# XUANTIE-RV/csi-nn2

Hardware: AMD Instinct MI355X
Metric: mobilenetv1_int8_images_per_sec (higher is better)
Workload: dtype i8; 1 GPU; mobilenetv1 int8 NHWC batch 1/GPU, 28 conv layers in 15 launches, hipGraph replay via csinn_*; ops_per_image=1137480704, algorithmic_bytes_per_image=8323144, algorithmic_bytes_per_image_survey=14444616, parallelism=replicas x1

## Files before the change

csi-nn2_amd/__init__.py:

```python
import ctypes as C
import os

import numpy as np

HERE = os.path.dirname(os.path.abspath(__file__))
ROOT = os.path.dirname(HERE)
LIB_DIR = os.path.join(HERE, "lib")

DTYPE_INT8, DTYPE_INT32, DTYPE_FLOAT16, DTYPE_FLOAT32 = 3, 7, 8, 10
MEM_CPU, MEM_DMABUF, MEM_CPU_ACC = 0, 2, 5
QUANT_INT8_ASYM_W_SYM, QUANT_FLOAT16 = 11, 7
API_REF, API_GREF, API_MI355X = 0, 1, 14
RM_LAYER, RM_CPU_GRAPH = 0, 1
LAYOUT_N, LAYOUT_NC, LAYOUT_NCHW, LAYOUT_O, LAYOUT_OI, LAYOUT_OIHW, LAYOUT_O1HW = 1, 2, 4, 6, 7, 11, 13
LAYOUT_NHWC, LAYOUT_OHWI, LAYOUT_1HWO = 15, 18, 22
CSINN_TRUE = 1
OP_CONV2D, OP_CONV2D_RELU, OP_CONV2D_RELU6 = 28, 29, 30
OP_DEPTHWISE_CONV2D, OP_FULLYCONNECTED = 35, 71

SHL_NHWC, SHL_NCHW = 0, 1
SHL_I8, SHL_F16 = 0, 1
ACT_NONE, ACT_RELU, ACT_RELU6 = 0, 1, 2
ALGO_AUTO, ALGO_DIRECT, ALGO_IGEMM, ALGO_DW, ALGO_GEMV, ALGO_STEM = 0, 1, 2, 3, 4, 5

# ... 155 lines not shown
        "shl_mi355x_comm_unique_id": (C.c_int, [vp]),
        "shl_mi355x_comm_create": (C.c_int, [vp, i32, i32, C.POINTER(vp)]),
        "shl_mi355x_comm_destroy": (C.c_int, [vp]),
        "shl_mi355x_comm_info": (C.c_int, [vp, C.POINTER(i32), C.POINTER(i32), C.POINTER(i32)]),
        "shl_mi355x_device_bus_id": (C.c_int, [C.c_char_p, sz]),
        "shl_mi355x_comm_bcast": (C.c_int, [vp, C.POINTER(vp), C.POINTER(sz), i32, i32, vp]),
        "shl_mi355x_conv_plan_destroy": (C.c_int, [vp]),
        "shl_mi355x_conv_plan_algo": (C.c_int, [vp]),
        "shl_mi355x_conv_plan_kernel_name": (C.c_char_p, [vp]),
        "shl_mi355x_conv_plan_bytes": (sz, [vp]),
        "shl_mi355x_conv_plan_const_block": (vp, [vp, C.POINTER(sz)]),
        "shl_mi355x_conv_plan_adopt_block": (C.c_int, [vp, vp]),
        "shl_mi355x_conv_forward": (C.c_int, [vp, vp, vp, i32, vp]),
        "shl_mi355x_pwdw_fusable": (C.c_int, [vp, vp, i32]),
        "shl_mi355x_pwdw_form": (C.c_int, [vp, vp, i32]),
        "shl_mi355x_pool_conv_fusable": (C.c_int, [vp, i32, i32]),
        "shl_mi355x_pool_conv_forward": (C.c_int, [vp, vp, vp, i32, i32, f32, i32, f32, i32, vp]),
        "shl_mi355x_conv_pool_fusable": (C.c_int, [vp, i32]),
        "shl_mi355x_conv_pool_forward": (C.c_int, [vp, vp, vp, vp, i32, f32, i32, f32, i32, vp]),
        "shl_mi355x_conv_plan_set_no_stream_consumer": (C.c_int, [vp, i32]),
        "shl_mi355x_pwdw_forward": (C.c_int, [vp, vp, vp, vp, i32, vp]),
        "shl_mi355x_relu_i8": (C.c_int, [vp, vp, sz, f32, i32, f32, i32, i32, vp]),
        "shl_mi355x_relu_f16": (C.c_int, [vp, vp, sz, i32, vp]),
        "shl_mi355x_add": (C.c_int, [vp, vp, vp, sz, i32, f32, i32, f32, i32, f32, i32, vp]),
        "shl_mi355x_layout_convert": (C.c_int, [vp, vp, C.c_int64, i32, i32, i32, i32, vp]),
        "shl_mi355x_global_avgpool2d": (C.c_int, [vp, vp, i32, i32, i32, i32, i32, f32, i32, f32, i32, vp]),
        "shl_mi355x_softmax": (C.c_int, [vp, vp, i32, C.c_int64, i32, C.c_int64, f32, i32, f32, i32, vp]),
    }
    for name, (res, args) in sigs.items():
        fn = getattr(lib, name)
# ... 213 lines not shown
```

csi-nn2_amd/csrc/common.h:

```cpp
#pragma once

#include <hip/hip_runtime.h>
#include <stdint.h>

#include "shl_mi355x.h"

namespace shl {

typedef int v4i __attribute__((ext_vector_type(4)));
typedef int v16i __attribute__((ext_vector_type(16)));
typedef float v16f __attribute__((ext_vector_type(16)));
typedef _Float16 v8h __attribute__((ext_vector_type(8)));

struct ConvArgs {
    const void *in;
    const void *w;
    void *out;
    const int32_t *acc_init;
    const float *mult;
    const float *bias;
    int32_t N, H, W, C;
    int32_t Ho, Wo, Co;
    int32_t Kh, Kw;
    int32_t sh, sw, pt, pl, dh, dw;
// ... 423 lines not shown
int launch_dwconv_channel(const ConvArgs &a, hipStream_t s);
bool conv_gemv_pick(const ConvArgs &a, int esize);
int launch_conv_gemv(const ConvArgs &a, int dtype, hipStream_t s);
bool pool_gemv_pick(const ConvArgs &a, int hw);
int launch_pool_gemv(const ConvArgs &a, int hw, float in_scale, int in_zp, float mid_scale, int mid_zp, hipStream_t s);
bool stem_supports(const shl_mi355x_conv_desc &d);
void stem_pack_weights(const shl_mi355x_conv_desc &d, const int8_t *ohwi, int32_t *dst);
size_t stem_weight_bytes(const shl_mi355x_conv_desc &d);
int launch_conv_stem(const ConvArgs &a, hipStream_t s);
bool conv1x1_nchw_eligible(const ConvArgs &a);
int launch_conv1x1_nchw(const ConvArgs &a, int dtype, hipStream_t s);
bool dwconv_nchw_supports(const shl_mi355x_conv_desc &d);
int launch_dwconv_nchw(const ConvArgs &a, int dtype, hipStream_t s);
bool pwdw_fusable(const ConvArgs &pw, const ConvArgs &dw, int pw_is_igemm, int dw_dot4_packed);
int launch_pwdw_fused(const ConvArgs &pw, const ConvArgs &dw, hipStream_t s);
bool stemdw_f16_nchw_fusable(const ConvArgs &stem, const ConvArgs &dw);
int launch_stemdw_f16_nchw(const ConvArgs &stem, const ConvArgs &dw, hipStream_t s);
bool stem_mfma_pick(const ConvArgs &a);
bool dwpw_stream_fusable(const ConvArgs &dw, const ConvArgs &pw, int dw_dot4_packed, int pw_is_igemm);
bool dwpw_stream_takes(const ConvArgs &dw);
int launch_dwpw_stream(const ConvArgs &dw, const ConvArgs &pw, hipStream_t s);
bool dwpw_resident_fusable(const ConvArgs &dw, const ConvArgs &pw, int dw_dot4_packed, int pw_is_igemm);
bool dwpw_resident_takes(const ConvArgs &dw);
int launch_dwpw_resident(const ConvArgs &dw, const ConvArgs &pw, hipStream_t s);
bool pwdw_f16_nchw_fusable(const ConvArgs &pw, const ConvArgs &dw);
int launch_pwdw_f16_nchw(const ConvArgs &pw, const ConvArgs &dw, hipStream_t s);
bool stemdw_fusable(const ConvArgs &stem, const ConvArgs &dw);
int launch_stemdw_fused(const ConvArgs &stem, const ConvArgs &dw, hipStream_t s);
bool patch_supports(const shl_mi355x_conv_desc &d);
int patch_choose_geom(const shl_mi355x_conv_desc &d, int32_t batch);
// ... 9 lines not shown
```

csi-nn2_amd/csrc/conv_plan.hip:

```cpp
#include <stdlib.h>
#include <string.h>

#include <map>
#include <mutex>
#include <vector>

#include "igemm_common.h"

struct shl_mi355x_conv_plan {
    shl_mi355x_conv_desc desc;
    int algo;
    char *block;
    size_t block_bytes;
    size_t off_w, off_acc, off_mult, off_bias, off_pad;
    size_t off_wfrag;
    size_t off_wpatch;
    size_t off_flags;
    int32_t pt_geom;
    int32_t div_exact, div_fma, act_clamp;
    float clamp_lo, clamp_hi, inv_out_scale;
    char *scratch_in, *scratch_out;
    int2 *pix_tab;
    float ch_in_scale, ch_out_scale;
    int32_t ch_has_bias;
// ... 984 lines not shown
    const bool i8_nhwc = pw->desc.dtype == SHL_MI355X_I8 && pw->desc.layout == SHL_MI355X_NHWC;
    const bool f16_nchw = pw->desc.dtype == SHL_MI355X_F16 && pw->desc.layout == SHL_MI355X_NCHW;
    if (!i8_nhwc && !f16_nchw) return 0;
    ConvArgs a, b;
    static char dummy[16];
    if (fill_args(pw, dummy, dummy, batch, a) != SHL_MI355X_OK || fill_args(dw, dummy, dummy, batch, b) != SHL_MI355X_OK)
        return 0;
    return pwdw_kernel_for(pw, dw, a, b);
}

int shl_mi355x_pwdw_fusable(const shl_mi355x_conv_plan *pw, const shl_mi355x_conv_plan *dw, int32_t batch)
{
    return shl_mi355x_pwdw_form(pw, dw, batch) ? 1 : 0;
}

int shl_mi355x_pwdw_forward(const shl_mi355x_conv_plan *pw, const shl_mi355x_conv_plan *dw, const void *input_dev,
                            void *output_dev, int32_t batch, void *stream)
{
    if (!dw || !pw || !input_dev || !output_dev) {
        set_error("pwdw_forward: NULL argument");
        return SHL_MI355X_EINVAL;
    }
    if (!shl_mi355x_pwdw_fusable(pw, dw, batch)) {
        set_error("pwdw_forward: the pair does not qualify for the fused kernel");
        return SHL_MI355X_ENOTSUP;
    }
    ConvArgs a, b;
    int rc = fill_args(pw, input_dev, output_dev, batch, a);
    if (rc == SHL_MI355X_OK) rc = fill_args(dw, input_dev, output_dev, batch, b);
    if (rc != SHL_MI355X_OK) return rc;
// ... 13 lines not shown
```

csi-nn2_amd/csrc/dw_patch.h:

```cpp
#pragma once

#include <stddef.h>

#include "common.h"

namespace shl {

__device__ __forceinline__ int dw_patch_slot(int j, int group, int pitch) { return group * pitch + j; }
__host__ __device__ __forceinline__ int dw_patch_pitch(int npx) { return ((npx + 31) & ~31) + 8; }
__host__ __device__ __forceinline__ size_t dw_patch_bytes(int npx) { return (size_t)dw_patch_pitch(npx) * 32; }
__device__ __forceinline__ uint32_t dw_patch_pad(const ConvArgs &d) { return (uint32_t)(d.in_zp & 0xff) * 0x01010101u; }

template <class T>
__device__ __forceinline__ T kernarg_here(size_t off)
{
    typedef const __attribute__((address_space(4))) char *KernargPtr;
    KernargPtr p = (KernargPtr)__builtin_amdgcn_kernarg_segment_ptr();
    asm volatile("" : "+s"(p));
    T v;
    __builtin_memcpy(&v, (const __attribute__((address_space(4))) T *)(p + off), sizeof(T));
    return v;
}

struct DwPatchGeom {
    int bh, bw;
    int rw;
    int pitch;
    uint32_t bw_magic;
    int oy0, ox0;
    int ry0, rx0;
    int n;
    int ch0;
};

struct DwThreadConsts {
    uint4 w0, w1, w2;
    int4 ai;
    float4 mu, bi;
};

// ... 18 lines not shown
struct DwPrep {
    int8_t *out_img;
    int nout;
    int po;
    DwOutPos first;
};

__device__ __forceinline__ DwOutPos dw_patch_locate(const ConvArgs &d, const DwPatchGeom &g, int cg, int po)
{
    const int oyl = (int)(((uint32_t)po * g.bw_magic) >> 20);
    const int oxl = po - oyl * g.bw;
    const int oy = g.oy0 + oyl, ox = g.ox0 + oxl;
    DwOutPos p;
    p.lds = (uint32_t)(cg * g.pitch + (oyl * d.sh) * g.rw + oxl * d.sw);
    p.out = (uint32_t)((oy * d.Wo + ox) * d.C + g.ch0 + cg * 4);
    p.live = oy < d.Ho && ox < d.Wo;
    return p;
}

__device__ __forceinline__ DwPrep dw_patch_prepare(const ConvArgs &d, const DwPatchGeom &g, int tid)
{
    DwPrep p;
    p.out_img = static_cast<int8_t *>(d.out) + (g.n ? (int64_t)g.n * d.Ho * d.Wo * d.C : (int64_t)0);
    p.nout = g.bh * g.bw;
    p.po = tid >> 3;
    p.first = dw_patch_locate(d, g, tid & 7, p.po);
    const uint32_t live = p.first.live ? 1u : 0u;
    asm volatile("" ::"s"(p.out_img), "s"(p.nout), "v"(p.po), "v"(p.first.lds), "v"(p.first.out), "v"(live));
    p.first.live = live != 0;
    return p;
}
// ... 43 lines not shown
```

csi-nn2_amd/csrc/pwdw_fused.hip:

```cpp
#include <stdio.h>
#include <stdlib.h>

#include "dw_patch.h"
#include "igemm_common.h"

namespace shl {

struct PwDwArgs {
    ConvArgs pw;
    ConvArgs dw;
    int32_t bh, bw;
    int32_t tiles_x, tiles_y;
    int32_t rw;
    int32_t npx;
    int32_t mt;
    int32_t nwaves;
    int32_t ks;
    int32_t nsw;
    int32_t nsub;
    uint32_t rw_magic;
    uint32_t bw_magic;
    int32_t xg, xg_log2;
    int32_t spg;
    uint32_t spg_magic;
    uint32_t tx_magic;
    int32_t nrect;
    int32_t ks_log2;
    int32_t mwn;
    int64_t img_stride;
};

template <int MTW, int NSW, int MAXT, bool EXACT, int KSV = 0, int TPW = 0, bool EMT = false, int EPQ = -1, int EPD = -1>
__global__ __launch_bounds__(MAXT) void pwdw_fused_kernel(PwDwArgs f)
{
    static_assert((KSV == 0) == (TPW == 0) && (TPW == 0 || (TPW == MTW && EXACT)), "pwdw_fused: KSV and TPW come together, with MTW = TPW");
    constexpr bool FIXED = TPW != 0;
    extern __shared__ __attribute__((aligned(16))) char smem[];
    const ConvArgs &q = f.pw;
    const ConvArgs &d = f.dw;
    const int tid = threadIdx.x;
    const int lane = tid & 63;
    const int wave = __builtin_amdgcn_readfirstlane(tid >> 6);
    const int frow = lane & 31, fhalf = lane >> 5;
    asm volatile("" ::"s"(f.xg), "s"(f.xg_log2), "s"(f.spg), "s"(f.spg_magic), "s"(f.tx_magic), "s"(f.nrect), "s"(f.tiles_x), "s"(f.tiles_y));
    asm volatile("" ::"s"(f.bh), "s"(f.bw), "s"(f.rw), "s"(f.npx), "s"(f.mt), "s"(f.ks), "s"(f.nsw), "s"(f.nsub), "s"(f.rw_magic),
                 "s"(f.ks_log2), "s"(f.mwn), "s"(f.img_stride));
    asm volatile("" ::"s"(q.in), "s"(q.w_frag), "s"(q.H), "s"(q.W), "s"(q.C), "s"(d.sh), "s"(d.sw), "s"(d.pt), "s"(d.pl), "s"(d.N));
    int slice = blockIdx.x, tx = blockIdx.y, ty = blockIdx.z, n = 0;
    {
        const int L = blockIdx.x;
        const int x = L & 7, j = L >> 3;
        const int b = (int)(((uint32_t)j * f.spg_magic) >> 20);
        const int xslice = (x & (f.xg - 1)) * f.spg + (j - b * f.spg);
        const int rect = b * (8 >> f.xg_log2) + (x >> f.xg_log2);
        const int xty = (int)(((uint32_t)rect * f.tx_magic) >> 20);
        const int xtx = rect - xty * f.tiles_x;
        const bool mapped = f.xg != 0;
        if (mapped && rect >= f.nrect) return;
        slice = mapped ? xslice : slice;
        ty = mapped ? xty : ty;
        tx = mapped ? xtx : tx;
    }
    if (d.N > 1) {
        n = ty / f.tiles_y;
        ty -= n * f.tiles_y;
    }
    const int oy0 = ty * f.bh, ox0 = tx * f.bw;
    const int ry0 = oy0 * d.sh - d.pt, rx0 = ox0 * d.sw - d.pl;

    const int nwaves = FIXED ? 4 : f.nwaves;
    const int fgrp = wave & 3;

    const int ks = FIXED ? KSV : f.ks;
    const int kpart = wave & (ks - 1);
    const int mw = wave >> (FIXED ? (KSV == 4 ? 2 : (KSV == 2 ? 1 : 0)) : f.ks_log2);
    const int mwn = FIXED ? 4 / (KSV ? KSV : 1) : f.mwn;
    const int mtp = FIXED ? TPW * (4 / (KSV ? KSV : 1)) : f.mt;
    const int mt = (FIXED && EMT) ? mtp : f.mt;
    const int sub0 = kpart * f.nsw;
    int nsw = NSW;
    if constexpr (!EXACT) {
        nsw = f.nsub - sub0;
        nsw = nsw < f.nsw ? nsw : f.nsw;
    }

    const char *img = static_cast<const char *>(q.in) + (n ? (int64_t)n * f.img_stride : (int64_t)0);
    const char *wp = static_cast<const char *>(q.w_frag) + ((int64_t)slice * f.nsub + sub0) * 1024 + lane * 16;
    constexpr int wstep = 1024;
    v4i fa[NSW];
#pragma unroll
    for (int s = 0; s < NSW; ++s)
        if (s < nsw) fa[s] = *reinterpret_cast<const v4i *>(wp + s * wstep);
    if constexpr (FIXED) __builtin_amdgcn_sched_barrier(0);
    v4i fb[MTW][NSW];
#pragma unroll
    for (int i = 0; i < MTW; ++i) {
        const int tile = mw + i * mwn;
        if (FIXED || tile < mt) {
            int j = tile * 32 + frow;
            j = j < f.npx ? j : f.npx - 1;
            const int r = (int)(((uint32_t)j * f.rw_magic) >> 20);
            const int c = j - r * f.rw;
            int y = ry0 + r, x = rx0 + c;
            y = max(0, min(y, q.H - 1));
            x = max(0, min(x, q.W - 1));
            const char *px = img + (y * q.W + x) * q.C + fhalf * 16 + sub0 * 32;
#pragma unroll
            for (int s = 0; s < NSW; ++s)
                if (s < nsw) fb[i][s] = *reinterpret_cast<const v4i *>(px + s * 32);
        }
    }
    __builtin_amdgcn_sched_barrier(0);
    const uint32_t bw_magic = kernarg_here<uint32_t>(offsetof(PwDwArgs, bw_magic));
    const ConvArgs ql = kernarg_here<ConvArgs>(offsetof(PwDwArgs, pw)), dl = kernarg_here<ConvArgs>(offsetof(PwDwArgs, dw));
    asm volatile("" ::"s"(ql.acc_init), "s"(ql.mult), "s"(ql.bias), "s"(ql.out_zp), "s"(ql.out_zp_f), "s"(ql.clamp_lo), "s"(ql.clamp_hi),
                 "s"(ql.out_scale), "s"(ql.inv_out_scale), "s"(dl.w), "s"(dl.acc_init), "s"(dl.mult), "s"(dl.bias), "s"(dl.out));
    asm volatile("" ::"s"(dl.out_zp), "s"(dl.out_zp_f), "s"(dl.clamp_lo), "s"(dl.clamp_hi), "s"(dl.out_scale), "s"(dl.inv_out_scale),
                 "s"(dl.in_zp), "s"(dl.Ho), "s"(dl.Wo), "s"(dl.C), "s"(dl.sh), "s"(dl.sw), "s"(bw_magic));
    const int pc = slice * 32 + 8 * fgrp + 4 * fhalf;
    const int4 p_ai = *reinterpret_cast<const int4 *>(ql.acc_init + pc);
    const float4 p_mu = *reinterpret_cast<const float4 *>(ql.mult + pc);
    const float4 p_bi = *reinterpret_cast<const float4 *>(ql.bias + pc);

    const DwThreadConsts dwk = dw_load_consts(dl, slice * 32, tid);
    DwPatchGeom g;
    g.bh = f.bh, g.bw = f.bw, g.rw = f.rw, g.bw_magic = bw_magic, g.pitch = dw_patch_pitch(f.npx);
    g.oy0 = oy0, g.ox0 = ox0, g.ry0 = ry0, g.rx0 = rx0, g.n = n, g.ch0 = slice * 32;
    const DwPrep dwp = dw_patch_prepare(dl, g, tid);
    const int ppitch = g.pitch;
    const uint32_t zpad = dw_patch_pad(dl);
    {
        const float qcl = ql.clamp_lo - ql.out_zp_f, qch = ql.clamp_hi - ql.out_zp_f, dcl = dl.clamp_lo - dl.out_zp_f, dch = dl.clamp_hi - dl.out_zp_f;
        const uint32_t qzp2 = (uint32_t)(ql.out_zp & 0xffff) * 0x00010001u, dzp2 = (uint32_t)(dl.out_zp & 0xffff) * 0x00010001u;
        asm volatile("" ::"s"(ppitch), "s"(zpad), "v"(qcl), "v"(qch), "v"(dcl), "v"(dch), "s"(qzp2), "s"(dzp2));
    }
    auto in_image = [&](int j) {
        const int r = (int)(((uint32_t)j * f.rw_magic) >> 20);
        const int c = j - r * f.rw;
        return (unsigned)(ry0 + r) < (unsigned)q.H && (unsigned)(rx0 + c) < (unsigned)q.W;
    };
    constexpr int NFT = (FIXED && EMT) ? TPW * (4 / (KSV ? KSV : 1)) : 1;
    uint32_t fslot[NFT], fkeep[NFT];
    if constexpr (FIXED && EMT) {
#pragma unroll
        for (int t = 0; t < NFT; ++t) {
            const int j = t * 32 + frow;
            fslot[t] = (uint32_t)dw_patch_slot(j, 2 * fgrp + fhalf, ppitch);
            fkeep[t] = in_image(j) ? 0xffffffffu : 0u;
            asm volatile("" ::"v"(fslot[t]), "v"(fkeep[t]));
        }
    }
    __builtin_amdgcn_sched_barrier(0);

    v16i acc[MTW];
    if constexpr (EXACT) {
        const v16i zero16 = {0, 0, 0, 0, 0, 0, 0, 0, 0, 0, 0, 0, 0, 0, 0, 0};
#pragma unroll
        for (int s = 0; s < NSW; ++s) {
#pragma unroll
            for (int i = 0; i < MTW; ++i)
                if (FIXED || mw + i * mwn < mt) acc[i] = __builtin_amdgcn_mfma_i32_32x32x32_i8(fa[s], fb[i][s], s == 0 ? zero16 : acc[i], 0, 0, 0);
        }
    } else {
#pragma unroll
        for (int i = 0; i < MTW; ++i)
#pragma unroll
            for (int r = 0; r < 16; ++r) acc[i][r] = 0;
#pragma unroll
        for (int s = 0; s < NSW; ++s) {
            if (s < nsw) {
#pragma unroll
                for (int i = 0; i < MTW; ++i)
                    if (mw + i * mwn < mt) acc[i] = __builtin_amdgcn_mfma_i32_32x32x32_i8(fa[s], fb[i][s], acc[i], 0, 0, 0);
            }
        }
    }

    if constexpr (!FIXED)
        if (q.debug & 256) return;
    v4i *part = reinterpret_cast<v4i *>(smem);
    uint32_t *patch = reinterpret_cast<uint32_t *>(smem + (size_t)mtp * ks * 4096);
#pragma unroll
    for (int i = 0; i < MTW; ++i) {
        const int tile = mw + i * mwn;
        if (FIXED || tile < mt) {
#pragma unroll
            for (int g = 0; g < 4; ++g) {
                v4i v;
#pragma unroll
                for (int e = 0; e < 4; ++e) v[e] = acc[i][4 * g + e];
                part[((tile * ks + kpart) * 4 + g) * 64 + lane] = v;
            }
        }
    }
    __syncthreads();
    if constexpr (!FIXED)
        if (q.debug & 512) return;
    {
        auto put = [&](int tile, int j, uint32_t pk) {
            if constexpr (FIXED && EMT) {
                if (j < f.npx) patch[fslot[tile]] = (pk & fkeep[tile]) | (zpad & ~fkeep[tile]);
            } else {
                if (j < f.npx) patch[dw_patch_slot(j, 2 * fgrp + fhalf, ppitch)] = in_image(j) ? pk : zpad;
            }
        };
        const int tstep = nwaves >> 2;
        for (int tile = FIXED ? 0 : wave >> 2; tile < mt; tile += 2 * tstep) {
            const int tile1 = tile + tstep;
            const int j0 = tile * 32 + frow;
            v4i v0 = part[((tile * ks) * 4 + fgrp) * 64 + lane];
            if (tile1 < mt) {
                v4i v1 = part[((tile1 * ks) * 4 + fgrp) * 64 + lane];
#pragma unroll
                for (int k = 1; k < ks; ++k) {
                    v0 += part[((tile * ks + k) * 4 + fgrp) * 64 + lane];
                    v1 += part[((tile1 * ks + k) * 4 + fgrp) * 64 + lane];
                }
                const uint32_t pk0 = requant4_i8_sel<EPQ>(v0[0] + p_ai.x, v0[1] + p_ai.y, v0[2] + p_ai.z, v0[3] + p_ai.w, p_mu, p_bi, ql);
// ... 25 lines not shown
constexpr int PWDW_MTW = 4;

static bool shapes_pair(const ConvArgs &q, const ConvArgs &d)
{
    if (q.Kh != 1 || q.Kw != 1 || q.sh != 1 || q.sw != 1 || q.pt != 0 || q.pl != 0) return false;
    if (q.H != q.Ho || q.W != q.Wo || (q.C & 31) != 0 || (q.Co & 31) != 0 || q.kstride < q.C) return false;
    if (d.Kh != 3 || d.Kw != 3 || d.dh != 1 || d.dw != 1 || d.C != d.Co || d.C != q.Co) return false;
    if (d.H != q.Ho || d.W != q.Wo || d.N != q.N) return false;
    if (d.sh < 1 || d.sh > 2 || d.sw < 1 || d.sw > 2 || d.pt > 2 || d.pl > 2 || d.pt < 0 || d.pl < 0) return false;
    if (q.C > 1024 || !q.w_frag) return false;
    if ((int64_t)q.H * q.W * q.C >= ((int64_t)1 << 31)) return false;
    if ((int64_t)d.Ho * d.Wo * d.C >= ((int64_t)1 << 31)) return false;
    return true;
}

static bool choose_rect(const ConvArgs &q, const ConvArgs &d, PwDwArgs &f)
{
    const int nsub = q.C >> 5;
    const int nwaves = waves_per_group();
    const int ks = ks_for(nsub, nwaves);
    const int mt_max = (nwaves / ks) * PWDW_MTW;
    const int nsw = (nsub + ks - 1) / ks;
    if (nwaves == 8 && nsw > 4) return false;
    const int64_t slices = q.Co >> 5;
    int force_h = 0, force_w = 0;
    const char *env = getenv("SHL_MI355X_PWDW_TILE");
    if (env) sscanf(env, "%dx%d", &force_h, &force_w);
    double best = 1e30;
    int best_h = 0, best_w = 0;
    for (int bh = 1; bh <= d.Ho && bh <= 32; ++bh) {
        for (int div = 1; div <= 16; ++div) {
            const int bw = (d.Wo + div - 1) / div;
            if (div > 1 && bw == (d.Wo + div - 2) / (div - 1)) continue;
            if (force_h && (bh != force_h || bw != force_w)) continue;
            const int rh = (bh - 1) * d.sh + 3, rw = (bw - 1) * d.sw + 3;
            const int npx = rh * rw;
            const int mt = (npx + 31) / 32;
            if (mt > mt_max || rw > 256 || bw > 256 || npx >= 4096 || bh * bw >= 4096) continue;
            if ((size_t)mt * ks * 4096 + dw_patch_bytes(npx) > 96 * 1024) continue;
            const int64_t blocks = slices * ((d.Ho + bh - 1) / bh) * ((d.Wo + bw - 1) / bw) * d.N;
            const double rounds = (double)((blocks + 255) / 256);
            const double score = rounds * ((mt + 1) * nsub + 2.0 * ((bh * bw + 31) / 32) + 4.0) -
                                 (blocks <= 256 ? blocks / 1024.0 : 0.0);
            if (score < best) {
                best = score;
                best_h = bh;
                best_w = bw;
            }
        }
    }
    if (!best_h) return false;
    f.bh = best_h;
    f.bw = best_w;
    f.tiles_y = (d.Ho + f.bh - 1) / f.bh;
    f.tiles_x = (d.Wo + f.bw - 1) / f.bw;
    f.rw = (f.bw - 1) * d.sw + 3;
    f.npx = ((f.bh - 1) * d.sh + 3) * f.rw;
    f.mt = (f.npx + 31) / 32;
    f.nwaves = nwaves;
    f.ks = ks;
    f.nsw = nsw;
    f.nsub = nsub;
    f.ks_log2 = ks == 8 ? 3 : (ks == 4 ? 2 : (ks == 2 ? 1 : 0));
    f.mwn = nwaves / ks;
    f.img_stride = (int64_t)q.H * q.W * q.C;
    f.rw_magic = ((1u << 20) + f.rw - 1) / f.rw;
    f.bw_magic = ((1u << 20) + f.bw - 1) / f.bw;
    {
        const int S = (int)slices;
        const int64_t R = (int64_t)f.tiles_x * f.tiles_y * d.N;
        static const char *xe = getenv("SHL_MI355X_PWDW_XG");
        const int forced = xe ? atoi(xe) : -1;
        const double act = (double)q.N * q.H * q.W * q.C, wts = (double)q.C * q.Co;
        int best_g = 0;
        double best_c = 1e30;
        for (int g = 1; g <= 8; g <<= 1) {
            if (S % g) continue;
            if (forced > 0 && g != forced) continue;
            if (forced <= 0 && g > 1 && ((S / g) & 3) != 0) continue;
            const int rpg = 8 / g;
            const int64_t per_xcd = (int64_t)(S / g) * ((R + rpg - 1) / rpg);
            if (per_xcd >= 4096 || R >= 4096) continue;
// ... 11 lines not shown
    return true;
}

bool pwdw_fusable(const ConvArgs &q, const ConvArgs &d, int pw_is_igemm, int dw_dot4_packed)
{
    if (!pw_is_igemm || !dw_dot4_packed || !shapes_pair(q, d)) return false;
    PwDwArgs f;
    if (!choose_rect(q, d, f)) return false;
    if ((int64_t)f.tiles_y * d.N > 65535 || f.tiles_x > 65535) return false;
    static const char *sel = getenv("SHL_MI355X_PWDW");
    const int64_t blocks = (int64_t)(q.Co >> 5) * f.tiles_x * f.tiles_y * d.N;
    if (blocks > 512 && !(sel && sel[0] == '2')) return false;
    return true;
}

int launch_pwdw_fused(const ConvArgs &q, const ConvArgs &d, hipStream_t s)
{
    PwDwArgs f;
    f.pw = q;
    f.dw = d;
    if (!shapes_pair(q, d) || !choose_rect(q, d, f)) {
        set_error("pwdw_fused: the pair does not qualify");
        return SHL_MI355X_ENOTSUP;
    }
    dim3 grid((unsigned)(q.Co >> 5), (unsigned)f.tiles_x, (unsigned)(f.tiles_y * d.N));
    if (f.xg) {
        const int rpg = 8 / f.xg;
        grid = dim3((unsigned)(8 * f.spg * ((f.nrect + rpg - 1) / rpg)), 1, 1);
    }
    size_t lds = (size_t)f.mt * f.ks * 4096 + dw_patch_bytes(f.npx);
    {
        static const char *pr = getenv("SHL_MI355X_PWDW_PRINT");
        if (pr && pr[0] == '1')
            fprintf(stderr, "pwdw_fused %d->%d @%dx%d s%d: rect %dx%d, npx %d, mt %d, ks %d, nsw %d, nsub %d, mwn %d, xg %d, grid %u\n", q.C, q.Co, d.H, d.W,
                    d.sh, f.bh, f.bw, f.npx, f.mt, f.ks, f.nsw, f.nsub, f.mwn, f.xg, grid.x * grid.y * grid.z);
    }
#define SHL_PWDW2(NSWV, MAXT, EX)                                                                                    \
    do {                                                                                                       \
        static LdsOptIn opted_in;                                                                              \
        if (lds > 64 * 1024) lds_opt_in(opted_in, reinterpret_cast<const void *>(pwdw_fused_kernel<PWDW_MTW, NSWV, MAXT, EX>)); \
        hipLaunchKernelGGL((pwdw_fused_kernel<PWDW_MTW, NSWV, MAXT, EX>), grid, dim3(64 * f.nwaves), lds, s, f);               \
    } while (0)
#define SHL_PWDW(NSWV, MAXT)                                           \
    do {                                                              \
        if (f.nsw == NSWV && f.nsub == f.ks * NSWV) SHL_PWDW2(NSWV, MAXT, true); \
        else SHL_PWDW2(NSWV, MAXT, false);                            \
    } while (0)
    const int epq = (q.act != SHL_MI355X_ACT_NONE && !q.act_clamp) ? -1 : (q.div_exact ? 3 : 0);
    const int epd = (d.act != SHL_MI355X_ACT_NONE && !d.act_clamp) ? -1 : (d.div_exact ? 3 : 0);
#define SHL_PWDW_EPI(TPWV, NSWV, KSV, EMTV)                                                                              \
    do {                                                                                                                \
        if (epq == 3 && epd == 3)                                                                                       \
            hipLaunchKernelGGL((pwdw_fused_kernel<TPWV, NSWV, 512, true, KSV, TPWV, EMTV, 3, 3>), grid, dim3(256), lds, s, f); \
        else if (epq == 0 && epd == 0)                                                                                  \
            hipLaunchKernelGGL((pwdw_fused_kernel<TPWV, NSWV, 512, true, KSV, TPWV, EMTV, 0, 0>), grid, dim3(256), lds, s, f); \
        else                                                                                                            \
            hipLaunchKernelGGL((pwdw_fused_kernel<TPWV, NSWV, 512, true, KSV, TPWV, EMTV>), grid, dim3(256), lds, s, f);    \
    } while (0)
#define SHL_PWDW_FIXED(NSWV, KSV, TPWV)                                                                                  \
    if (f.nwaves == 4 && f.nsw == NSWV && f.nsub == KSV * NSWV && f.ks == KSV && f.mt <= TPWV * (4 / KSV) &&            \
        f.mt > (TPWV - 1) * (4 / KSV)) {                                                                                \
        lds = (size_t)(TPWV * (4 / KSV)) * f.ks * 4096 + dw_patch_bytes(f.npx);     \
        if (f.mt == TPWV * (4 / KSV))                                                                                   \
            SHL_PWDW_EPI(TPWV, NSWV, KSV, true);                                                                        \
        else                                                                                                            \
            SHL_PWDW_EPI(TPWV, NSWV, KSV, false);                                                                       \
        SHL_HIP(hipGetLastError());                                                                                     \
        return SHL_MI355X_OK;                                                                                           \
    }
    const char *nofix = getenv("SHL_MI355X_PWDW_GENERIC");
    if (!(nofix && nofix[0] == '1')) {
        SHL_PWDW_FIXED(4, 4, 2)
        SHL_PWDW_FIXED(4, 4, 1)
        SHL_PWDW_FIXED(2, 4, 2)
        SHL_PWDW_FIXED(2, 4, 1)
        SHL_PWDW_FIXED(2, 2, 2)
        SHL_PWDW_FIXED(2, 2, 1)
// ... 21 lines not shown
```

csi-nn2_amd/csrc/stemdw_fused.hip:

```cpp
#include <stdio.h>
#include <stdlib.h>

#include "dw_patch.h"

namespace shl {

struct StemDwArgs {
    ConvArgs st;
    ConvArgs dw;
    int32_t bh, bw;
    int32_t tiles_x, tiles_y;
    int32_t rw, npx;
    uint32_t rw_magic, bw_magic;
};

template <int EPQ, int EPD>
__global__ __launch_bounds__(256) void stemdw_fused_kernel(StemDwArgs f)
{
    extern __shared__ __attribute__((aligned(16))) char smem[];
    const ConvArgs &q = f.st;
    const ConvArgs &d = f.dw;
    asm volatile("" ::"s"(q.in), "s"(q.w), "s"(q.acc_init), "s"(q.mult), "s"(q.bias), "s"(q.H), "s"(q.W), "s"(q.Ho), "s"(q.Wo), "s"(q.sh),
                 "s"(q.sw), "s"(q.pt), "s"(q.pl), "s"(q.dh), "s"(q.dw), "s"(q.in_zp));
    asm volatile("" ::"s"(f.bh), "s"(f.bw), "s"(f.tiles_y), "s"(f.rw), "s"(f.npx), "s"(f.rw_magic), "s"(f.bw_magic), "s"(d.N), "s"(d.sh),
// ... 13 lines not shown
    int ty = blockIdx.y, n = 0;
    if (d.N > 1) {
        n = ty / f.tiles_y;
        ty -= n * f.tiles_y;
    }
    const int oy0 = ty * f.bh, ox0 = tx * f.bw;
    const int ry0 = oy0 * d.sh - d.pt, rx0 = ox0 * d.sw - d.pl;
    const DwThreadConsts dwk = dw_load_consts(d, 0, tid);

    const int8_t *img = static_cast<const int8_t *>(q.in) + (int64_t)n * q.H * q.W * 3;
    const int ntasks = 2 * f.npx;
    const int ppitch = dw_patch_pitch(f.npx);
    const uint32_t zpad = dw_patch_pad(d);
    DwPatchGeom g;
    g.bh = f.bh, g.bw = f.bw, g.rw = f.rw, g.bw_magic = f.bw_magic, g.pitch = ppitch;
    g.oy0 = oy0, g.ox0 = ox0, g.ry0 = ry0, g.rx0 = rx0, g.n = n, g.ch0 = 0;
    const DwPrep dwp = dw_patch_prepare(d, g, tid);
    for (int base = 0; base < ntasks; base += 256) {
        const bool valid = base + tid < ntasks;
        const int task = valid ? base + tid : ntasks - 1;
        const int j = task >> 1, cb = (task & 1) * 16;
        const int pr = (int)(((uint32_t)j * f.rw_magic) >> 20);
        const int pc = j - pr * f.rw;
        const int sy = ry0 + pr, sx = rx0 + pc;
        const bool inside = (unsigned)sy < (unsigned)q.Ho && (unsigned)sx < (unsigned)q.Wo;
        const int y0 = sy * q.sh - q.pt, x0 = sx * q.sw - q.pl;
        int qv[28];
#pragma unroll
        for (int ky = 0; ky < 3; ++ky)
#pragma unroll
// ... 94 lines not shown
```

include/shl_mi355x.h:

```cpp
#ifndef SHL_MI355X_H_
#define SHL_MI355X_H_

#include <stddef.h>
#include <stdint.h>

#ifdef __cplusplus
extern "C" {
#endif

#define SHL_MI355X_ABI_VERSION 1

enum shl_mi355x_status {
    SHL_MI355X_OK = 0,
    SHL_MI355X_ENODEV = -1,
    SHL_MI355X_EINVAL = -2,
    SHL_MI355X_ENOTSUP = -3,
    SHL_MI355X_EHIP = -4,
    SHL_MI355X_ENOMEM = -5
};

enum shl_mi355x_layout {
    SHL_MI355X_NHWC = 0,
    SHL_MI355X_NCHW = 1
};
// ... 102 lines not shown
void *shl_mi355x_conv_plan_const_block(shl_mi355x_conv_plan *plan, size_t *bytes);
int shl_mi355x_conv_plan_adopt_block(shl_mi355x_conv_plan *plan, void *stream);

int shl_mi355x_conv_forward(const shl_mi355x_conv_plan *plan, const void *input_dev,
                            void *output_dev, int32_t batch, void *stream);

int shl_mi355x_pool_conv_fusable(const shl_mi355x_conv_plan *plan, int32_t batch, int32_t pixels);
int shl_mi355x_pool_conv_forward(const shl_mi355x_conv_plan *plan, const void *input_dev, void *output_dev, int32_t batch,
                                 int32_t pixels, float in_scale, int32_t in_zp, float mid_scale, int32_t mid_zp, void *stream);
int shl_mi355x_conv_pool_fusable(const shl_mi355x_conv_plan *plan, int32_t batch);
int shl_mi355x_conv_pool_forward(const shl_mi355x_conv_plan *plan, const void *input_dev, void *map_dev, void *pool_dev, int32_t batch,
                                 float mid_scale, int32_t mid_zp, float out_scale, int32_t out_zp, void *stream);
int shl_mi355x_conv_plan_set_no_stream_consumer(shl_mi355x_conv_plan *plan, int32_t on);
int shl_mi355x_pwdw_fusable(const shl_mi355x_conv_plan *pw, const shl_mi355x_conv_plan *dw, int32_t batch);
int shl_mi355x_pwdw_form(const shl_mi355x_conv_plan *pw, const shl_mi355x_conv_plan *dw, int32_t batch);
int shl_mi355x_pwdw_forward(const shl_mi355x_conv_plan *pw, const shl_mi355x_conv_plan *dw,
                            const void *input_dev, void *output_dev, int32_t batch, void *stream);

int shl_mi355x_relu_i8(const int8_t *input_dev, int8_t *output_dev, size_t count,
                       float in_scale, int32_t in_zp, float out_scale, int32_t out_zp,
                       int32_t relu6, void *stream);

int shl_mi355x_relu_f16(const uint16_t *input_dev, uint16_t *output_dev, size_t count, int32_t relu6,
                        void *stream);

int shl_mi355x_add(const void *input0_dev, const void *input1_dev, void *output_dev, size_t count,
                   int32_t dtype, float scale0, int32_t zp0, float scale1, int32_t zp1, float out_scale,
                   int32_t out_zp, void *stream);

int shl_mi355x_global_avgpool2d(const void *input_dev, void *output_dev, int32_t dtype, int32_t layout,
// ... 15 lines not shown
```

Before: 18950 img/s.

## Allow non-uniform border tiles in fused pw+dw and compute only in-image windows

The fused pointwise+depthwise kernel's tile chooser now considers grids whose first and last tiles are one pixel larger, so output extents that do not divide evenly need no ragged partial tiles. The pointwise stage computes only the clipped in-image input window (nwin) instead of the full padded patch, which can lower the MFMA tile count, and padding is written into LDS up front rather than masked per pixel. A geometry query API is added for inspection. This adds more kernel-argument state, a prefill of the patch, and a more complex search over tile shapes.

```diff
diff --git a/csi-nn2_amd/__init__.py b/csi-nn2_amd/__init__.py
--- a/csi-nn2_amd/__init__.py
+++ b/csi-nn2_amd/__init__.py
@@ -193,6 +193,7 @@
         "shl_mi355x_conv_forward": (C.c_int, [vp, vp, vp, i32, vp]),
         "shl_mi355x_pwdw_fusable": (C.c_int, [vp, vp, i32]),
         "shl_mi355x_pwdw_form": (C.c_int, [vp, vp, i32]),
+        "shl_mi355x_pwdw_geometry": (C.c_int, [vp, vp, i32, C.POINTER(i32), i32]),
         "shl_mi355x_pool_conv_fusable": (C.c_int, [vp, i32, i32]),
         "shl_mi355x_pool_conv_forward": (C.c_int, [vp, vp, vp, i32, i32, f32, i32, f32, i32, vp]),
         "shl_mi355x_conv_pool_fusable": (C.c_int, [vp, i32]),
diff --git a/csi-nn2_amd/csrc/common.h b/csi-nn2_amd/csrc/common.h
--- a/csi-nn2_amd/csrc/common.h
+++ b/csi-nn2_amd/csrc/common.h
@@ -461,6 +461,8 @@
 int launch_dwconv_nchw(const ConvArgs &a, int dtype, hipStream_t s);
 bool pwdw_fusable(const ConvArgs &pw, const ConvArgs &dw, int pw_is_igemm, int dw_dot4_packed);
 int launch_pwdw_fused(const ConvArgs &pw, const ConvArgs &dw, hipStream_t s);
+constexpr int SHL_PWDW_GEOMETRY_FIELDS = 12;
+bool pwdw_fused_geometry(const ConvArgs &pw, const ConvArgs &dw, int32_t out[SHL_PWDW_GEOMETRY_FIELDS]);
 bool stemdw_f16_nchw_fusable(const ConvArgs &stem, const ConvArgs &dw);
 int launch_stemdw_f16_nchw(const ConvArgs &stem, const ConvArgs &dw, hipStream_t s);
 bool stem_mfma_pick(const ConvArgs &a);
diff --git a/csi-nn2_amd/csrc/conv_plan.hip b/csi-nn2_amd/csrc/conv_plan.hip
--- a/csi-nn2_amd/csrc/conv_plan.hip
+++ b/csi-nn2_amd/csrc/conv_plan.hip
@@ -1022,6 +1022,29 @@
     return shl_mi355x_pwdw_form(pw, dw, batch) ? 1 : 0;
 }
 
+int shl_mi355x_pwdw_geometry(const shl_mi355x_conv_plan *pw, const shl_mi355x_conv_plan *dw, int32_t batch, int32_t *out, int32_t count)
+{
+    using namespace shl;
+    if (!out || count < SHL_PWDW_GEOMETRY_FIELDS) {
+        set_error("pwdw_geometry: room for 12 values is needed");
+        return SHL_MI355X_EINVAL;
+    }
+    if (shl_mi355x_pwdw_form(pw, dw, batch) != 1) {
+        set_error("pwdw_geometry: the pair does not run the latency form");
+        return SHL_MI355X_ENOTSUP;
+    }
+    ConvArgs a, b;
+    static char dummy[16];
+    int rc = fill_args(pw, dummy, dummy, batch, a);
+    if (rc == SHL_MI355X_OK) rc = fill_args(dw, dummy, dummy, batch, b);
+    if (rc != SHL_MI355X_OK) return rc;
+    if (!pwdw_fused_geometry(a, b, out)) {
+        set_error("pwdw_geometry: the pair does not qualify");
+        return SHL_MI355X_ENOTSUP;
+    }
+    return SHL_MI355X_OK;
+}
+
 int shl_mi355x_pwdw_forward(const shl_mi355x_conv_plan *pw, const shl_mi355x_conv_plan *dw, const void *input_dev,
                             void *output_dev, int32_t batch, void *stream)
 {
diff --git a/csi-nn2_amd/csrc/dw_patch.h b/csi-nn2_amd/csrc/dw_patch.h
--- a/csi-nn2_amd/csrc/dw_patch.h
+++ b/csi-nn2_amd/csrc/dw_patch.h
@@ -24,6 +24,7 @@
 
 struct DwPatchGeom {
     int bh, bw;
+    int lbh, lbw;
     int rw;
     int pitch;
     uint32_t bw_magic;
@@ -72,7 +73,7 @@
     DwOutPos p;
     p.lds = (uint32_t)(cg * g.pitch + (oyl * d.sh) * g.rw + oxl * d.sw);
     p.out = (uint32_t)((oy * d.Wo + ox) * d.C + g.ch0 + cg * 4);
-    p.live = oy < d.Ho && ox < d.Wo;
+    p.live = oyl < g.lbh && oxl < g.lbw;
     return p;
 }
 
diff --git a/csi-nn2_amd/csrc/pwdw_fused.hip b/csi-nn2_amd/csrc/pwdw_fused.hip
--- a/csi-nn2_amd/csrc/pwdw_fused.hip
+++ b/csi-nn2_amd/csrc/pwdw_fused.hip
@@ -1,25 +1,35 @@
 #include <stdio.h>
 #include <stdlib.h>
 
+#include <algorithm>
+#include <vector>
+
 #include "dw_patch.h"
 #include "igemm_common.h"
 
 namespace shl {
+
+struct alignas(32) PwDwLateArgs {
+    uint32_t bw_magic;
+    int32_t rw;
+    int32_t npx;
+    int32_t dbh, dbw;
+    int32_t bhe, bwe;
+    int32_t ylast, xlast;
+    int32_t cy, cx;
+    int32_t reserved;
+};
 
 struct PwDwArgs {
     ConvArgs pw;
     ConvArgs dw;
     int32_t bh, bw;
     int32_t tiles_x, tiles_y;
-    int32_t rw;
-    int32_t npx;
     int32_t mt;
     int32_t nwaves;
     int32_t ks;
     int32_t nsw;
     int32_t nsub;
-    uint32_t rw_magic;
-    uint32_t bw_magic;
     int32_t xg, xg_log2;
     int32_t spg;
     uint32_t spg_magic;
@@ -28,13 +38,21 @@
     int32_t ks_log2;
     int32_t mwn;
     int64_t img_stride;
+    int32_t ex_lo, ex_hi, ey_lo, ey_hi;
+    int32_t iwm;
+    uint32_t iwm_magic;
+    int32_t nwin;
+    PwDwLateArgs late;
 };
+
+constexpr int PWDW_PAD_DWORDS = 3;
 
 template <int MTW, int NSW, int MAXT, bool EXACT, int KSV = 0, int TPW = 0, bool EMT = false, int EPQ = -1, int EPD = -1>
 __global__ __launch_bounds__(MAXT) void pwdw_fused_kernel(PwDwArgs f)
 {
     static_assert((KSV == 0) == (TPW == 0) && (TPW == 0 || (TPW == MTW && EXACT)), "pwdw_fused: KSV and TPW come together, with MTW = TPW");
     constexpr bool FIXED = TPW != 0;
+    constexpr int NFT_ALL = FIXED ? TPW * (4 / (KSV ? KSV : 1)) : 1;
     extern __shared__ __attribute__((aligned(16))) char smem[];
     const ConvArgs &q = f.pw;
     const ConvArgs &d = f.dw;
@@ -43,9 +61,10 @@
     const int wave = __builtin_amdgcn_readfirstlane(tid >> 6);
     const int frow = lane & 31, fhalf = lane >> 5;
     asm volatile("" ::"s"(f.xg), "s"(f.xg_log2), "s"(f.spg), "s"(f.spg_magic), "s"(f.tx_magic), "s"(f.nrect), "s"(f.tiles_x), "s"(f.tiles_y));
-    asm volatile("" ::"s"(f.bh), "s"(f.bw), "s"(f.rw), "s"(f.npx), "s"(f.mt), "s"(f.ks), "s"(f.nsw), "s"(f.nsub), "s"(f.rw_magic),
+    asm volatile("" ::"s"(f.bh), "s"(f.bw), "s"(f.mt), "s"(f.ks), "s"(f.nsw), "s"(f.nsub),
                  "s"(f.ks_log2), "s"(f.mwn), "s"(f.img_stride));
     asm volatile("" ::"s"(q.in), "s"(q.w_frag), "s"(q.H), "s"(q.W), "s"(q.C), "s"(d.sh), "s"(d.sw), "s"(d.pt), "s"(d.pl), "s"(d.N));
+    asm volatile("" ::"s"(f.ex_lo), "s"(f.ey_lo), "s"(f.iwm), "s"(f.iwm_magic));
     int slice = blockIdx.x, tx = blockIdx.y, ty = blockIdx.z, n = 0;
     {
         const int L = blockIdx.x;
@@ -65,8 +84,6 @@
         n = ty / f.tiles_y;
         ty -= n * f.tiles_y;
     }
-    const int oy0 = ty * f.bh, ox0 = tx * f.bw;
-    const int ry0 = oy0 * d.sh - d.pt, rx0 = ox0 * d.sw - d.pl;
 
     const int nwaves = FIXED ? 4 : f.nwaves;
     const int fgrp = wave & 3;
@@ -92,18 +109,21 @@
     for (int s = 0; s < NSW; ++s)
         if (s < nsw) fa[s] = *reinterpret_cast<const v4i *>(wp + s * wstep);
     if constexpr (FIXED) __builtin_amdgcn_sched_barrier(0);
+    const int oy0 = ty * f.bh + min(ty, f.ey_lo), ox0 = tx * f.bw + min(tx, f.ex_lo);
+    const int ry0 = oy0 * d.sh - d.pt, rx0 = ox0 * d.sw - d.pl;
+    const int wy0 = max(ry0, 0), wx0 = max(rx0, 0);
+    auto win_rc = [&](int j, int &r, int &c) {
+        r = (int)(((uint32_t)j * f.iwm_magic) >> 20);
+        c = j - r * f.iwm;
+    };
     v4i fb[MTW][NSW];
+    int lr[MTW], lc[MTW];
 #pragma unroll
     for (int i = 0; i < MTW; ++i) {
         const int tile = mw + i * mwn;
         if (FIXED || tile < mt) {
-            int j = tile * 32 + frow;
-            j = j < f.npx ? j : f.npx - 1;
-            const int r = (int)(((uint32_t)j * f.rw_magic) >> 20);
-            const int c = j - r * f.rw;
-            int y = ry0 + r, x = rx0 + c;
-            y = max(0, min(y, q.H - 1));
-            x = max(0, min(x, q.W - 1));
+            win_rc(tile * 32 + frow, lr[i], lc[i]);
+            const int y = min(wy0 + lr[i], q.H - 1), x = min(wx0 + lc[i], q.W - 1);
             const char *px = img + (y * q.W + x) * q.C + fhalf * 16 + sub0 * 32;
 #pragma unroll
             for (int s = 0; s < NSW; ++s)
@@ -111,20 +131,23 @@
         }
     }
     __builtin_amdgcn_sched_barrier(0);
-    const uint32_t bw_magic = kernarg_here<uint32_t>(offsetof(PwDwArgs, bw_magic));
+    const PwDwLateArgs fl = kernarg_here<PwDwLateArgs>(offsetof(PwDwArgs, late));
+    const uint32_t bw_magic = fl.bw_magic;
     const ConvArgs ql = kernarg_here<ConvArgs>(offsetof(PwDwArgs, pw)), dl = kernarg_here<ConvArgs>(offsetof(PwDwArgs, dw));
     asm volatile("" ::"s"(ql.acc_init), "s"(ql.mult), "s"(ql.bias), "s"(ql.out_zp), "s"(ql.out_zp_f), "s"(ql.clamp_lo), "s"(ql.clamp_hi),
                  "s"(ql.out_scale), "s"(ql.inv_out_scale), "s"(dl.w), "s"(dl.acc_init), "s"(dl.mult), "s"(dl.bias), "s"(dl.out));
     asm volatile("" ::"s"(dl.out_zp), "s"(dl.out_zp_f), "s"(dl.clamp_lo), "s"(dl.clamp_hi), "s"(dl.out_scale), "s"(dl.inv_out_scale),
                  "s"(dl.in_zp), "s"(dl.Ho), "s"(dl.Wo), "s"(dl.C), "s"(dl.sh), "s"(dl.sw), "s"(bw_magic));
+    asm volatile("" ::"s"(fl.bhe), "s"(fl.bwe), "s"(fl.cy), "s"(fl.cx), "s"(fl.ylast), "s"(fl.xlast), "s"(fl.dbh), "s"(fl.dbw), "s"(fl.rw), "s"(fl.npx));
     const int pc = slice * 32 + 8 * fgrp + 4 * fhalf;
     const int4 p_ai = *reinterpret_cast<const int4 *>(ql.acc_init + pc);
     const float4 p_mu = *reinterpret_cast<const float4 *>(ql.mult + pc);
     const float4 p_bi = *reinterpret_cast<const float4 *>(ql.bias + pc);
 
     const DwThreadConsts dwk = dw_load_consts(dl, slice * 32, tid);
+    const int oye = ty == fl.ylast ? dl.Ho : ty * f.bh + fl.bhe, oxe = tx == fl.xlast ? dl.Wo : tx * f.bw + fl.bwe;
     DwPatchGeom g;
-    g.bh = f.bh, g.bw = f.bw, g.rw = f.rw, g.bw_magic = bw_magic, g.pitch = dw_patch_pitch(f.npx);
+    g.bh = fl.dbh, g.bw = fl.dbw, g.lbh = oye - oy0, g.lbw = oxe - ox0, g.rw = fl.rw, g.bw_magic = bw_magic, g.pitch = dw_patch_pitch(fl.npx);
     g.oy0 = oy0, g.ox0 = ox0, g.ry0 = ry0, g.rx0 = rx0, g.n = n, g.ch0 = slice * 32;
     const DwPrep dwp = dw_patch_prepare(dl, g, tid);
     const int ppitch = g.pitch;
@@ -134,23 +157,32 @@
         const uint32_t qzp2 = (uint32_t)(ql.out_zp & 0xffff) * 0x00010001u, dzp2 = (uint32_t)(dl.out_zp & 0xffff) * 0x00010001u;
         asm volatile("" ::"s"(ppitch), "s"(zpad), "v"(qcl), "v"(qch), "v"(dcl), "v"(dch), "s"(qzp2), "s"(dzp2));
     }
-    auto in_image = [&](int j) {
-        const int r = (int)(((uint32_t)j * f.rw_magic) >> 20);
-        const int c = j - r * f.rw;
-        return (unsigned)(ry0 + r) < (unsigned)q.H && (unsigned)(rx0 + c) < (unsigned)q.W;
-    };
+    __builtin_amdgcn_sched_barrier(0);
+
+    const int wye = min(oye * dl.sh + fl.cy, q.H), wxe = min(oxe * dl.sw + fl.cx, q.W);
+    const int wslot0 = (wy0 - ry0) * fl.rw + (wx0 - rx0) + (2 * fgrp + fhalf) * ppitch;
+    auto win_has = [&](int r, int c) { return wy0 + r < wye && wx0 + c < wxe; };
+    auto win_slot = [&](int r, int c) { return (uint32_t)(wslot0 + r * fl.rw + c); };
     constexpr int NFT = (FIXED && EMT) ? TPW * (4 / (KSV ? KSV : 1)) : 1;
-    uint32_t fslot[NFT], fkeep[NFT];
+    uint32_t fslot[NFT];
     if constexpr (FIXED && EMT) {
+        const uint32_t spare = (uint32_t)((2 * fgrp + fhalf) * ppitch + ppitch - 1);
 #pragma unroll
         for (int t = 0; t < NFT; ++t) {
-            const int j = t * 32 + frow;
-            fslot[t] = (uint32_t)dw_patch_slot(j, 2 * fgrp + fhalf, ppitch);
-            fkeep[t] = in_image(j) ? 0xffffffffu : 0u;
-            asm volatile("" ::"v"(fslot[t]), "v"(fkeep[t]));
-        }
-    }
-    __builtin_amdgcn_sched_barrier(0);
+            int r, c;
+            if constexpr (KSV == 4) r = lr[t], c = lc[t];
+            else win_rc(t * 32 + frow, r, c);
+            fslot[t] = win_has(r, c) ? win_slot(r, c) : spare;
+            asm volatile("" ::"v"(fslot[t]));
+        }
+    }
+    uint32_t *patch = reinterpret_cast<uint32_t *>(smem + (size_t)mtp * ks * 4096);
+    if constexpr (FIXED) {
+#pragma unroll
+        for (int k = 0; k < PWDW_PAD_DWORDS * NFT_ALL; ++k) patch[tid + 256 * k] = zpad;
+    } else {
+        for (int i = tid; i < 8 * ppitch; i += nwaves * 64) patch[i] = zpad;
+    }
 
     v16i acc[MTW];
     if constexpr (EXACT) {
@@ -179,7 +211,6 @@
     if constexpr (!FIXED)
         if (q.debug & 256) return;
     v4i *part = reinterpret_cast<v4i *>(smem);
-    uint32_t *patch = reinterpret_cast<uint32_t *>(smem + (size_t)mtp * ks * 4096);
 #pragma unroll
     for (int i = 0; i < MTW; ++i) {
         const int tile = mw + i * mwn;
@@ -199,9 +230,11 @@
     {
         auto put = [&](int tile, int j, uint32_t pk) {
             if constexpr (FIXED && EMT) {
-                if (j < f.npx) patch[fslot[tile]] = (pk & fkeep[tile]) | (zpad & ~fkeep[tile]);
+                patch[fslot[tile]] = pk;
             } else {
-                if (j < f.npx) patch[dw_patch_slot(j, 2 * fgrp + fhalf, ppitch)] = in_image(j) ? pk : zpad;
+                int r, c;
+                win_rc(j, r, c);
+                if (win_has(r, c)) patch[win_slot(r, c)] = pk;
             }
         };
         const int tstep = nwaves >> 2;
@@ -257,6 +290,36 @@
     return true;
 }
 
+struct PwDwAxis {
+    int b, n, e_lo, e_hi;
+    int win;
+};
+static int axis_window(int in_len, int out_len, int s, int pad, const PwDwAxis &a)
+{
+    int best = 0;
+    for (int t = 0; t < a.n; ++t) {
+        const int o0 = t * a.b + (t > 0 ? a.e_lo : 0);
+        const int len = std::min(a.b + (t == 0 ? a.e_lo : 0) + (t == a.n - 1 ? a.e_hi : 0), out_len - o0);
+        const int r0 = o0 * s - pad;
+        best = std::max(best, std::min(r0 + (len - 1) * s + 3, in_len) - std::max(r0, 0));
+    }
+    return best;
+}
+static std::vector<PwDwAxis> axis_grids(int in_len, int out_len, int s, int pad, const std::vector<int> &lens, int max_n, bool uniform_only)
+{
+    std::vector<PwDwAxis> v;
+    for (int b : lens) v.push_back({b, (out_len + b - 1) / b, 0, 0, 0});
+    if (!uniform_only)
+        for (int n = 2; n <= max_n && n <= out_len; ++n)
+            for (int e = 1; e <= 3; ++e) {
+                const int e_lo = e & 1, e_hi = e >> 1, rest = out_len - e_lo - e_hi;
+                if (rest < n || rest % n) continue;
+                v.push_back({rest / n, n, e_lo, e_hi, 0});
+            }
+    for (PwDwAxis &a : v) a.win = axis_window(in_len, out_len, s, pad, a);
+    return v;
+}
+
 static bool choose_rect(const ConvArgs &q, const ConvArgs &d, PwDwArgs &f)
 {
     const int nsub = q.C >> 5;
@@ -269,37 +332,53 @@
     int force_h = 0, force_w = 0;
     const char *env = getenv("SHL_MI355X_PWDW_TILE");
     if (env) sscanf(env, "%dx%d", &force_h, &force_w);
+    std::vector<int> lens_y, lens_x;
+    for (int bh = 1; bh <= d.Ho && bh <= 32; ++bh)
+        if (!force_h || bh == force_h) lens_y.push_back(bh);
+    for (int div = 1; div <= 16; ++div) {
+        const int bw = (d.Wo + div - 1) / div;
+        if (div > 1 && bw == (d.Wo + div - 2) / (div - 1)) continue;
+        if (!force_h || bw == force_w) lens_x.push_back(bw);
+    }
+    const std::vector<PwDwAxis> gy = axis_grids(q.H, d.Ho, d.sh, d.pt, lens_y, 32, force_h != 0);
+    const std::vector<PwDwAxis> gx = axis_grids(q.W, d.Wo, d.sw, d.pl, lens_x, 16, force_h != 0);
     double best = 1e30;
-    int best_h = 0, best_w = 0;
-    for (int bh = 1; bh <= d.Ho && bh <= 32; ++bh) {
-        for (int div = 1; div <= 16; ++div) {
-            const int bw = (d.Wo + div - 1) / div;
-            if (div > 1 && bw == (d.Wo + div - 2) / (div - 1)) continue;
-            if (force_h && (bh != force_h || bw != force_w)) continue;
-            const int rh = (bh - 1) * d.sh + 3, rw = (bw - 1) * d.sw + 3;
+    const PwDwAxis *best_y = nullptr, *best_x = nullptr;
+    for (const PwDwAxis &y : gy) {
+        for (const PwDwAxis &x : gx) {
+            const int dbh = y.b + std::max(y.e_lo, y.e_hi), dbw = x.b + std::max(x.e_lo, x.e_hi);
+            const int rh = (dbh - 1) * d.sh + 3, rw = (dbw - 1) * d.sw + 3;
             const int npx = rh * rw;
-            const int mt = (npx + 31) / 32;
-            if (mt > mt_max || rw > 256 || bw > 256 || npx >= 4096 || bh * bw >= 4096) continue;
+            const int nwin = std::max(y.win, 1) * std::max(x.win, 1);
+            const int mt = (nwin + 31) / 32;
+            if (dbh > 32 || mt > mt_max || rw > 256 || dbw > 256 || npx >= 4096 || dbh * dbw >= 4096) continue;
             if ((size_t)mt * ks * 4096 + dw_patch_bytes(npx) > 96 * 1024) continue;
-            const int64_t blocks = slices * ((d.Ho + bh - 1) / bh) * ((d.Wo + bw - 1) / bw) * d.N;
+            const int64_t blocks = slices * y.n * x.n * d.N;
             const double rounds = (double)((blocks + 255) / 256);
-            const double score = rounds * ((mt + 1) * nsub + 2.0 * ((bh * bw + 31) / 32) + 4.0) -
-                                 (blocks <= 256 ? blocks / 1024.0 : 0.0);
+            const double score = rounds * ((mt + 1) * nsub + 2.0 * ((dbh * dbw + 31) / 32) + 4.0) -
+                                 (blocks <= 256 ? blocks / 1024.0 : 0.0) + nwin * 1e-7;
             if (score < best) {
                 best = score;
-                best_h = bh;
-                best_w = bw;
+                best_y = &y;
+                best_x = &x;
             }
         }
     }
-    if (!best_h) return false;
-    f.bh = best_h;
-    f.bw = best_w;
-    f.tiles_y = (d.Ho + f.bh - 1) / f.bh;
-    f.tiles_x = (d.Wo + f.bw - 1) / f.bw;
-    f.rw = (f.bw - 1) * d.sw + 3;
-    f.npx = ((f.bh - 1) * d.sh + 3) * f.rw;
-    f.mt = (f.npx + 31) / 32;
+    if (!best_y) return false;
+    f.bh = best_y->b, f.ey_lo = best_y->e_lo, f.ey_hi = best_y->e_hi, f.tiles_y = best_y->n;
+    f.bw = best_x->b, f.ex_lo = best_x->e_lo, f.ex_hi = best_x->e_hi, f.tiles_x = best_x->n;
+    f.late.dbh = f.bh + std::max(f.ey_lo, f.ey_hi);
+    f.late.dbw = f.bw + std::max(f.ex_lo, f.ex_hi);
+    f.late.bhe = f.bh + f.ey_lo, f.late.bwe = f.bw + f.ex_lo;
+    f.late.ylast = f.tiles_y - 1, f.late.xlast = f.tiles_x - 1;
+    f.late.reserved = 0;
+    f.iwm = std::max(best_x->win, 1);
+    f.iwm_magic = ((1u << 20) + f.iwm - 1) / f.iwm;
+    f.late.cy = 3 - d.sh - d.pt, f.late.cx = 3 - d.sw - d.pl;
+    f.late.rw = (f.late.dbw - 1) * d.sw + 3;
+    f.late.npx = ((f.late.dbh - 1) * d.sh + 3) * f.late.rw;
+    f.nwin = std::max(best_y->win, 1) * std::max(best_x->win, 1);
+    f.mt = (f.nwin + 31) / 32;
     f.nwaves = nwaves;
     f.ks = ks;
     f.nsw = nsw;
@@ -307,8 +386,7 @@
     f.ks_log2 = ks == 8 ? 3 : (ks == 4 ? 2 : (ks == 2 ? 1 : 0));
     f.mwn = nwaves / ks;
     f.img_stride = (int64_t)q.H * q.W * q.C;
-    f.rw_magic = ((1u << 20) + f.rw - 1) / f.rw;
-    f.bw_magic = ((1u << 20) + f.bw - 1) / f.bw;
+    f.late.bw_magic = ((1u << 20) + f.late.dbw - 1) / f.late.dbw;
     {
         const int S = (int)slices;
         const int64_t R = (int64_t)f.tiles_x * f.tiles_y * d.N;
@@ -350,6 +428,16 @@
     return true;
 }
 
+bool pwdw_fused_geometry(const ConvArgs &q, const ConvArgs &d, int32_t out[SHL_PWDW_GEOMETRY_FIELDS])
+{
+    PwDwArgs f;
+    if (!shapes_pair(q, d) || !choose_rect(q, d, f)) return false;
+    const int32_t v[SHL_PWDW_GEOMETRY_FIELDS] = {f.tiles_y, f.tiles_x, f.bh,  f.bw, f.ey_lo, f.ey_hi,
+                                                 f.ex_lo,   f.ex_hi,   f.mt,  f.ks, f.nwin,  (int32_t)((q.Co >> 5) * f.nrect)};
+    for (int i = 0; i < SHL_PWDW_GEOMETRY_FIELDS; ++i) out[i] = v[i];
+    return true;
+}
+
 int launch_pwdw_fused(const ConvArgs &q, const ConvArgs &d, hipStream_t s)
 {
     PwDwArgs f;
@@ -364,12 +452,13 @@
         const int rpg = 8 / f.xg;
         grid = dim3((unsigned)(8 * f.spg * ((f.nrect + rpg - 1) / rpg)), 1, 1);
     }
-    size_t lds = (size_t)f.mt * f.ks * 4096 + dw_patch_bytes(f.npx);
+    size_t lds = (size_t)f.mt * f.ks * 4096 + dw_patch_bytes(f.late.npx);
     {
         static const char *pr = getenv("SHL_MI355X_PWDW_PRINT");
         if (pr && pr[0] == '1')
-            fprintf(stderr, "pwdw_fused %d->%d @%dx%d s%d: rect %dx%d, npx %d, mt %d, ks %d, nsw %d, nsub %d, mwn %d, xg %d, grid %u\n", q.C, q.Co, d.H, d.W,
-                    d.sh, f.bh, f.bw, f.npx, f.mt, f.ks, f.nsw, f.nsub, f.mwn, f.xg, grid.x * grid.y * grid.z);
+            fprintf(stderr, "pwdw_fused %d->%d @%dx%d s%d: %dx%d rects of %dx%d (+%d/+%d, +%d/+%d at the borders), npx %d, nwin %d, mt %d, ks %d, nsw %d, nsub %d, mwn %d, xg %d, grid %u\n",
+                    q.C, q.Co, d.H, d.W, d.sh, f.tiles_y, f.tiles_x, f.bh, f.bw, f.ey_lo, f.ey_hi, f.ex_lo, f.ex_hi, f.late.npx, f.nwin, f.mt, f.ks, f.nsw, f.nsub,
+                    f.mwn, f.xg, grid.x * grid.y * grid.z);
     }
 #define SHL_PWDW2(NSWV, MAXT, EX)                                                                                    \
     do {                                                                                                       \
@@ -395,8 +484,9 @@
     } while (0)
 #define SHL_PWDW_FIXED(NSWV, KSV, TPWV)                                                                                  \
     if (f.nwaves == 4 && f.nsw == NSWV && f.nsub == KSV * NSWV && f.ks == KSV && f.mt <= TPWV * (4 / KSV) &&            \
-        f.mt > (TPWV - 1) * (4 / KSV)) {                                                                                \
-        lds = (size_t)(TPWV * (4 / KSV)) * f.ks * 4096 + dw_patch_bytes(f.npx);     \
+        f.mt > (TPWV - 1) * (4 / KSV) && dw_patch_bytes(f.late.npx) <= (size_t)1024 * PWDW_PAD_DWORDS * (TPWV * (4 / KSV))) {                                                                         \
+                                               \
+        lds = (size_t)(TPWV * (4 / KSV)) * (f.ks * 4096 + 1024 * PWDW_PAD_DWORDS);                                        \
         if (f.mt == TPWV * (4 / KSV))                                                                                   \
             SHL_PWDW_EPI(TPWV, NSWV, KSV, true);                                                                        \
         else                                                                                                            \
diff --git a/csi-nn2_amd/csrc/stemdw_fused.hip b/csi-nn2_amd/csrc/stemdw_fused.hip
--- a/csi-nn2_amd/csrc/stemdw_fused.hip
+++ b/csi-nn2_amd/csrc/stemdw_fused.hip
@@ -51,6 +51,7 @@
     const uint32_t zpad = dw_patch_pad(d);
     DwPatchGeom g;
     g.bh = f.bh, g.bw = f.bw, g.rw = f.rw, g.bw_magic = f.bw_magic, g.pitch = ppitch;
+    g.lbh = min(f.bh, d.Ho - oy0), g.lbw = min(f.bw, d.Wo - ox0);
     g.oy0 = oy0, g.ox0 = ox0, g.ry0 = ry0, g.rx0 = rx0, g.n = n, g.ch0 = 0;
     const DwPrep dwp = dw_patch_prepare(d, g, tid);
     for (int base = 0; base < ntasks; base += 256) {
diff --git a/include/shl_mi355x.h b/include/shl_mi355x.h
--- a/include/shl_mi355x.h
+++ b/include/shl_mi355x.h
@@ -140,6 +140,7 @@
 int shl_mi355x_conv_plan_set_no_stream_consumer(shl_mi355x_conv_plan *plan, int32_t on);
 int shl_mi355x_pwdw_fusable(const shl_mi355x_conv_plan *pw, const shl_mi355x_conv_plan *dw, int32_t batch);
 int shl_mi355x_pwdw_form(const shl_mi355x_conv_plan *pw, const shl_mi355x_conv_plan *dw, int32_t batch);
+int shl_mi355x_pwdw_geometry(const shl_mi355x_conv_plan *pw, const shl_mi355x_conv_plan *dw, int32_t batch, int32_t *out, int32_t count);
 int shl_mi355x_pwdw_forward(const shl_mi355x_conv_plan *pw, const shl_mi355x_conv_plan *dw,
                             const void *input_dev, void *output_dev, int32_t batch, void *stream);
 
```

After: 19500 img/s, median of 6. 1.03x the previous value.
